# quarterwave0/LithographySimulator

Hardware: AMD Instinct MI355X
Metric: Abbe source-points x image-pixels per second (higher is better)
Workload: dtype f32

## Files before the change

lithographysimulator_amd/csrc/abbe_plan.hpp:

```cpp
#pragma once
#include <climits>
#include <cstddef>
#include <cstdint>
#include <cstdlib>
#include <initializer_list>

#include "../../include/litho_abbe.h"

#ifdef __HIPCC__
#define LITHO_HD __host__ __device__
#else
#define LITHO_HD
#endif

namespace litho {

struct PassGeom {
    int pn, c, N;
    int nt;
    int tcl;
    int kx0, kx1;
    int ky0, ky1;
    int rows;
    int general;
    int rect_off;
    int gcombine;
    int row_pairs;
    int coop_dma;
    unsigned xmask, ymask;
    long long t_point;
};

LITHO_HD constexpr unsigned natural_in_mask(int RL)
{
    return RL == 0 ? 0xF01Fu : RL == 1 ? 0xC007u : RL == 2 ? 0x8003u : 0xFFFFu;
}
LITHO_HD constexpr unsigned out_mask(int RL)
{
    return RL == 1 ? 0xF00Fu : RL == 2 ? 0xC003u : 0xFFFFu;
}

static constexpr int PLAN_WORDS = 14;

static constexpr int COARSE_PLANES = 4;
static constexpr int EDGE_MAX = 128;
static constexpr int GAM_CHUNKS = 1024;
static constexpr size_t GAM_PARTIAL = (size_t)GAM_CHUNKS * 2 * 2 * EDGE_MAX;
static inline size_t gam_float2(int pn) { return GAM_PARTIAL + 2 * 2 * EDGE_MAX + 2 * (size_t)pn; }
static constexpr size_t SIZEOF_FLOAT2 = 8;

struct EdgeGeom {
    int pn, c, h;
    int lo[2], len[2];
};

#ifndef LITHO_G_CAP
#define LITHO_G_CAP 128
#endif
static inline int g_cap(int pn)
{
    const size_t one = (size_t)((pn + 3) / 4) * 4 * pn * sizeof(float);
    size_t n = ((size_t)128 << 20) / one;
    return n < 8 ? 8 : (n > LITHO_G_CAP ? LITHO_G_CAP : (int)n);
}
static constexpr int SLAB_FLUSH_BATCHES = 64;
static constexpr size_t T_BUDGET_MAX = (size_t)1 << 30;
static constexpr size_t T_BUDGET_BIG = (size_t)4 << 30;
static constexpr size_t T_BUDGET_MIN = (size_t)256 << 20;

static inline size_t align_up(size_t v, size_t a) { return (v + a - 1) / a * a; }

static inline size_t general_item_bytes(int pn) { return (size_t)((pn + 3) / 4) * (size_t)pn * 4 * SIZEOF_FLOAT2; }

static inline size_t t_budget(int pn)
{
    const size_t one_general = general_item_bytes(pn);
    size_t b = 64 * one_general;
    if (b < T_BUDGET_MIN) b = T_BUDGET_MIN;
    const size_t cap = pn >= 4096 ? T_BUDGET_BIG : T_BUDGET_MAX;
    if (b > cap) b = cap;
    if (b < one_general + one_general / 2) b = one_general + one_general / 2;
    return b;
}

static inline bool coarse_eligible(int pn, int N)
{
    return N == 2 * pn && (pn == 256 || pn == 512 || pn == 1024 || pn == 2048 || pn == 4096);
}
static inline size_t ic_bytes(int pn, int N) { return coarse_eligible(pn, N) ? (size_t)COARSE_PLANES * pn * pn * sizeof(float) : 0; }
static inline size_t chat_bytes(int pn, int N) { return coarse_eligible(pn, N) ? (size_t)pn * pn * SIZEOF_FLOAT2 : 0; }
static inline size_t gam_bytes(int pn, int N) { return coarse_eligible(pn, N) ? gam_float2(pn) * SIZEOF_FLOAT2 : 0; }

static inline int embedded_size(int pn, int N)
{
    if (pn == N || 2 * pn == N || (pn & 1)) return pn;
    if (2 * pn < N) return N / 2 >= 256 ? N / 2 : pn;
    return N >= 1024 ? N : pn;
}
static inline size_t embed_extra_bytes(int pe)
{
    const size_t e = (size_t)pe * pe;
    return align_up(e * SIZEOF_FLOAT2, 256) + align_up(COARSE_PLANES * e * SIZEOF_FLOAT2, 256) + align_up(COARSE_PLANES * e * sizeof(float), 256);
}

struct Region {
    size_t off, bytes;
    size_t end() const { return off + bytes; }
};
struct WsLayout {
    Region plan;
    Region twtab;
    Region twtab2;
    Region slab;
    Region ic;
    Region chat;
    Region gam;
    Region T;
    size_t total;
};
static inline WsLayout ws_layout(int pn, int N)
{
    const size_t nt = (pn + 3) / 4;
    WsLayout l;
    size_t p = 0;
    l.plan = {p, 256}; p += 256;
    l.twtab = {p, (size_t)N * SIZEOF_FLOAT2}; p += align_up((size_t)N * SIZEOF_FLOAT2, 256);
    l.twtab2 = {p, (size_t)pn * SIZEOF_FLOAT2}; p += align_up((size_t)pn * SIZEOF_FLOAT2, 256);
    l.slab = {p, (size_t)g_cap(pn) * nt * 4 * pn * sizeof(float)}; p += align_up(l.slab.bytes, 256);
    l.ic = {p, ic_bytes(pn, N)}; p += align_up(l.ic.bytes, 256);
    l.chat = {p, chat_bytes(pn, N)}; p += align_up(l.chat.bytes, 256);
    l.gam = {p, gam_bytes(pn, N)}; p += align_up(l.gam.bytes, 256);
    l.T = {p, t_budget(pn)}; p += align_up(l.T.bytes, 256);
    l.total = p;
    return l;
}
static inline size_t workspace_bytes_at(int pn, int N) { return ws_layout(pn, N).total; }
static inline size_t workspace_bytes(int pn, int N)
{
    const size_t own = workspace_bytes_at(pn, N);
    const int pe = embedded_size(pn, N);
    if (pe == pn) return own;
    const size_t emb = workspace_bytes_at(pe, N) + embed_extra_bytes(pe);
    return own > emb ? own : emb;
}

static inline int check_sizes(int pn, int N)
{
    if (pn < 2 || pn > 16384 || (pn & 1)) return LITHO_E_ARG;
    if (N < 16 || N > 16384 || (N & (N - 1))) return LITHO_E_ARG;
    if (N < pn) return LITHO_E_NSMALL;
    return LITHO_OK;
}

static inline int ilog2(int v) { int l = 0; while ((1 << l) < v) ++l; return l; }

static inline int env_int(const char* name, int dflt)
{
    const char* e = getenv(name);
    return (e && *e) ? atoi(e) : dflt;
}

struct Knobs {
    int force_generic, force_general, groups, batch, xchunk, tile, w64, w64_8192, w64x, plane_chunk, xsplit, rect, xrect, coarse, gcombine, rowpairs, poison, embed, split, coopdma;
    static int pick(const litho_abbe_options* o, size_t off, const char* name, int dflt)
    {
        if (o && off + sizeof(int32_t) <= (size_t)o->size) {
            const int32_t v = *(const int32_t*)((const unsigned char*)o + off);
            if (v >= 0) return v;
        }
        return env_int(name, dflt);
    }
    static Knobs read(const litho_abbe_options* o)
    {
#define LITHO_KNOB(field, name, dflt) k.field = pick(o, offsetof(litho_abbe_options, field), name, dflt)
        Knobs k;
        LITHO_KNOB(force_generic, "LITHO_ABBE_FORCE_GENERIC", 0);
        LITHO_KNOB(force_general, "LITHO_ABBE_FORCE_GENERAL", 0);
        LITHO_KNOB(groups, "LITHO_ABBE_GROUPS", 0);
        LITHO_KNOB(batch, "LITHO_ABBE_BATCH", 0);
        LITHO_KNOB(xchunk, "LITHO_ABBE_XCHUNK", 0);
        LITHO_KNOB(tile, "LITHO_ABBE_TILE", 0);
        LITHO_KNOB(w64, "LITHO_ABBE_W64", 1);
        LITHO_KNOB(w64_8192, "LITHO_ABBE_W64_8192", 1);
        LITHO_KNOB(w64x, "LITHO_ABBE_W64X", 0);
        LITHO_KNOB(plane_chunk, "LITHO_ABBE_PLANE_CHUNK", 0);
        LITHO_KNOB(xsplit, "LITHO_ABBE_XSPLIT", 1);
        LITHO_KNOB(rect, "LITHO_ABBE_RECT", 1);
        LITHO_KNOB(xrect, "LITHO_ABBE_XRECT", 1);
        LITHO_KNOB(coarse, "LITHO_ABBE_COARSE", 1);
        LITHO_KNOB(gcombine, "LITHO_ABBE_GCOMBINE", 1);
        LITHO_KNOB(rowpairs, "LITHO_ABBE_ROWPAIRS", 0);
        LITHO_KNOB(poison, "LITHO_ABBE_POISON", 0);
// ... 305 lines not shown
```

lithographysimulator_amd/csrc/engine_kernels.hpp:

```cpp
#pragma once
#include <hip/hip_runtime.h>

#include "engine_common.hpp"
#include "abbe_plan.hpp"
#include "fft_core.hpp"
#include "wave_fft.hpp"

namespace litho {

template <int LOG2N>
struct Launch {
    using F = LineFFT<LOG2N, +1>;
    static constexpr int L = (F::T >= 64) ? 1 : 64 / F::T;
    static constexpr int THREADS = F::T * L;
#ifndef LITHO_NBUF
#define LITHO_NBUF 1
#endif
    static constexpr int NBUF = (LOG2N <= 12) ? LITHO_NBUF : 1;
    static constexpr size_t LDS_EXCH = (size_t)L * NBUF * F::LDS_LINE;
    static constexpr size_t LDS_BYTES = sizeof(float2) * (LDS_EXCH + F::LDS_TW);
#ifndef LITHO_WG_PER_CU
#define LITHO_WG_PER_CU 3
#endif
    static constexpr int WG_PER_CU = LOG2N <= 12 ? LITHO_WG_PER_CU : (LOG2N == 13 ? 2 : 1);
    static constexpr int WAVES = (THREADS / 256 > 0 ? THREADS / 256 : 1) * WG_PER_CU;
};


typedef unsigned int u32x2 __attribute__((ext_vector_type(2)));
static constexpr unsigned BUF_OOB = 0xFFFF0000u;

__device__ __forceinline__ __amdgpu_buffer_rsrc_t make_rsrc(const void* base, size_t bytes) {
    return __builtin_amdgcn_make_buffer_rsrc(const_cast<void*>(base), 0, (int)(unsigned)bytes, 0x00020000);
}
__device__ __forceinline__ float2 buf_load_c64(__amdgpu_buffer_rsrc_t r, unsigned off) {
    const u32x2 v = __builtin_amdgcn_raw_buffer_load_b64(r, off, 0, 0);
    return make_float2(__uint_as_float(v.x), __uint_as_float(v.y));
}
#ifndef LITHO_XSTORE_AUX
#define LITHO_XSTORE_AUX 16
#endif
template <int LOG2N> inline constexpr int t_store_aux = LOG2N >= 11 ? LITHO_XSTORE_AUX : 0;
typedef unsigned int u32x4 __attribute__((ext_vector_type(4)));
template <int AUX = 0>
__device__ __forceinline__ void buf_store_c64x2(__amdgpu_buffer_rsrc_t r, unsigned off, float2 a, float2 b) {
    u32x4 w;
    w.x = __float_as_uint(a.x); w.y = __float_as_uint(a.y);
    w.z = __float_as_uint(b.x); w.w = __float_as_uint(b.y);
    __builtin_amdgcn_raw_buffer_store_b128(w, r, off, 0, AUX);
}
template <int AUX = 0>
__device__ __forceinline__ void buf_store_c64(__amdgpu_buffer_rsrc_t r, unsigned off, float2 v) {
    u32x2 w;
    w.x = __float_as_uint(v.x);
    w.y = __float_as_uint(v.y);
    __builtin_amdgcn_raw_buffer_store_b64(w, r, off, 0, AUX);
}

__device__ __forceinline__ unsigned t_offset(const PassGeom& g, unsigned a, unsigned q) {
    return ((((q >> g.tcl) * g.rows + a) << g.tcl) + (q & ((1u << g.tcl) - 1u)));
}

typedef unsigned int uint2v __attribute__((ext_vector_type(2)));

__device__ __forceinline__ void touch_vgpr(float2& v) { asm volatile("" : "+v"(v.x), "+v"(v.y)); }
__device__ __forceinline__ void diag_keep(float2 v, unsigned o) { asm volatile("" ::"v"(v.x), "v"(v.y), "v"(o)); }

__device__ __forceinline__ const float* pack_weights() { return nullptr; }
__device__ __forceinline__ const float* pack_weights(const float* w) { return w; }

template <int LOG2N, int RL, bool PRUNED, int NP, int RP = 1, typename... Wt>
__global__ __launch_bounds__(Launch<LOG2N>::THREADS, (RP == 2 ? Launch<LOG2N>::WAVES / Launch<LOG2N>::WG_PER_CU * 2 : Launch<LOG2N>::WAVES)) void k_xpass_abbe(
    const float2* __restrict__ P, const float2* __restrict__ M, const int* __restrict__ shifts,
    float2* __restrict__ Tbuf, const float2* __restrict__ twtab, PassGeom g, int nb, int chunk, Wt... wts)
{
    constexpr bool WT = sizeof...(Wt) != 0;
    static_assert(sizeof...(Wt) <= 1 && !(WT && RP == 2), "weighted x-pass: one weight list, one row per workgroup (a weighted call ignores the row-pair knob)");
    [[maybe_unused]] const float* weights = pack_weights(wts...);
    using F = LineFFT<LOG2N, +1>;
    using LC = Launch<LOG2N>;
    constexpr unsigned IN = PRUNED ? natural_in_mask(RL) : 0xFFFFu;
    constexpr unsigned OUT = out_mask(RL);
    extern __shared__ __attribute__((aligned(16))) unsigned char smem_raw[];
    float2* smem = reinterpret_cast<float2*>(smem_raw);
    const int lt = threadIdx.x % F::T, lg = threadIdx.x / F::T;
    float2* lds = smem + (size_t)lg * LC::NBUF * F::LDS_LINE;

    typename F::Twiddles tw;
    F::load_twiddles(tw, twtab, lt, smem + LC::LDS_EXCH, threadIdx.x, LC::THREADS);

    static_assert(RP == 1 || (RP == 2 && NP == 1 && LC::L == 1), "row pairs: one plane, one line per workgroup");
    int a;
    if constexpr (LC::L == 1) {
        const int b = blockIdx.x, xcd = b & 7, i = b >> 3;
        a = ((i >> 2) * 32 + xcd * 4 + (i & 3)) * RP;
    } else {
        a = blockIdx.x * LC::L + lg;
    }
    const bool active = a < g.rows;
    const bool active1 = a + 1 < g.rows;
    const int r = g.ky0 + g.c + a;
    const size_t plane_bytes = (size_t)g.pn * g.pn * sizeof(float2);
    const __amdgpu_buffer_rsrc_t rM = make_rsrc(M, plane_bytes);

    unsigned koff[16];
    float2 pv[NP * RP][16];
    static_for<0, 16>([&](auto e_) {
        constexpr int e = decltype(e_)::value;
        if constexpr ((IN >> e) & 1u) {
            int k;
            const bool ok = centred_index(lt + F::T * e, F::N, g.kx0, g.kx1, k) && active;
            koff[e] = ok ? (unsigned)(g.c + k) : BUF_OOB;
        }
    });
    static_for<0, NP * RP>([&](auto p_) {
        constexpr int p = decltype(p_)::value;
        const __amdgpu_buffer_rsrc_t rP = make_rsrc(P + (size_t)(RP == 1 ? p : 0) * g.pn * g.pn, plane_bytes);
        static_for<0, 16>([&](auto e_) {
            constexpr int e = decltype(e_)::value;
            if constexpr ((IN >> e) & 1u)
                pv[p][e] = buf_load_c64(rP, koff[e] != BUF_OOB ? ((unsigned)(r + (RP == 1 ? 0 : p)) * g.pn + koff[e]) * 8u : BUF_OOB);
        });
    });
    unsigned toff[16];
    static_for<0, 16>([&](auto m_) {
        constexpr int m = decltype(m_)::value;
        if constexpr ((OUT >> m) & 1u) {
            int u;
            const bool ok = centred_index(lt + F::T * m, F::N, -g.c, g.pn - g.c, u) && active;
            const unsigned q = (unsigned)(u + g.c);
            toff[m] = ok ? t_offset(g, a, q) * 8u : BUF_OOB;
        }
    });

    const int s_begin = blockIdx.y * chunk;
    const int s_end = min(nb, s_begin + chunk);
    auto load_window = [&](int s, int rr, float2 (&mv)[16]) {
        const int dy = shifts[2 * s], dx = shifts[2 * s + 1];
        const unsigned mrow = (unsigned)(r + rr + dy) * g.pn + dx;
        static_for<0, 16>([&](auto e_) {
            constexpr int e = decltype(e_)::value;
            if constexpr ((IN >> e) & 1u)
#ifdef LITHO_DIAG_XNOLOAD
                mv[e] = make_float2((float)((mrow + koff[e]) & 1023u), 1.0f);
#else
                mv[e] = buf_load_c64(rM, koff[e] != BUF_OOB ? (mrow + koff[e]) * 8u : BUF_OOB);
#endif
        });
    };

    int flip = 0;
    float2 mnext[16];
    [[maybe_unused]] float wnext = 1.f;
    if (s_begin < s_end) load_window(s_begin, 0, mnext);
    if constexpr (WT) { if (s_begin < s_end) wnext = weights[s_begin]; }
    static_for<0, 16>([&](auto e_) {
        constexpr int e = decltype(e_)::value;
        if constexpr ((IN >> e) & 1u) touch_vgpr(mnext[e]);
    });
    const unsigned row1 = active1 ? (8u << g.tcl) : 0x80000000u;
    float2 held[RP == 2 ? 16 : 1];
    const bool hi8 = (threadIdx.x & 8) != 0;
    unsigned offc = 0, offd = 0;
    if constexpr (RP == 2) {
        const unsigned tileb = (unsigned)g.rows * (8u << g.tcl);
        offc = hi8 ? row1 - tileb : 0u;
        offd = hi8 ? 0u : row1 + tileb;
    }
    for (int s = s_begin; s < s_end; ++s) {
        static_for<0, RP>([&](auto rr_) {
            constexpr int rr = decltype(rr_)::value;
            float2 mv[16];
            static_for<0, 16>([&](auto e_) {
                constexpr int e = decltype(e_)::value;
                if constexpr ((IN >> e) & 1u) mv[e] = mnext[e];
            });
            [[maybe_unused]] float amp = 1.f;
            if constexpr (WT) amp = sqrtf(wnext);
#ifndef LITHO_XPASS_NO_PREFETCH
            if constexpr (rr + 1 < RP) load_window(s, rr + 1, mnext);
            else load_window(s + 1 < s_end ? s + 1 : s, 0, mnext);
#else
            if constexpr (rr + 1 < RP) load_window(s, rr + 1, mnext);
            else if (s + 1 < s_end) load_window(s + 1, 0, mnext);
#endif
            if constexpr (WT) {
                wnext = weights[s + 1 < s_end ? s + 1 : s];
                static_for<0, 16>([&](auto e_) {
                    constexpr int e = decltype(e_)::value;
                    if constexpr ((IN >> e) & 1u) mv[e] = make_float2(amp * mv[e].x, amp * mv[e].y);
                });
            }
            static_for<0, NP>([&](auto p_) {
                constexpr int p = decltype(p_)::value;
                float2 x[16];
                static_for<0, 16>([&](auto e_) {
                    constexpr int e = decltype(e_)::value;
                    if constexpr ((IN >> e) & 1u) x[e] = cmul(pv[RP == 1 ? p : rr][e], mv[e]);
                    else x[e] = make_float2(0.f, 0.f);
                });
                F::template run<LC::NBUF>(x, tw, lds, lt, flip);
                const __amdgpu_buffer_rsrc_t rT =
                    make_rsrc(Tbuf + ((size_t)p * nb + s) * g.t_point, (size_t)g.t_point * sizeof(float2));
                if constexpr (RP == 2 && rr == 0) {
                    static_for<0, 16>([&](auto m_) { held[decltype(m_)::value] = x[decltype(m_)::value]; });
                } else {
                    static_for<0, 16>([&](auto m_) {
                        constexpr int m = decltype(m_)::value;
#ifdef LITHO_DIAG_XNOSTORE
                        if constexpr ((OUT >> m) & 1u) diag_keep(x[m], toff[m]);
#elif defined(LITHO_DIAG_XSTORE_L2)
                        if constexpr ((OUT >> m) & 1u) buf_store_c64(rT, toff[m] == BUF_OOB ? BUF_OOB : (toff[m] & 0xFFFFFu), x[m]);
#else
                        if constexpr ((OUT >> m) & 1u) {
                            if constexpr (RP == 2) {
                                if (active) {
                                    const float bx = __uint_as_float(__builtin_amdgcn_update_dpp(0u, __float_as_uint(x[m].x), 0x128, 0xF, 0xF, false));
                                    const float by = __uint_as_float(__builtin_amdgcn_update_dpp(0u, __float_as_uint(x[m].y), 0x128, 0xF, 0xF, false));
                                    buf_store_c64<t_store_aux<LOG2N>>(rT, toff[m] + offc, hi8 ? make_float2(bx, by) : held[m]);
                                    buf_store_c64<t_store_aux<LOG2N>>(rT, toff[m] + offd, hi8 ? held[m] : make_float2(bx, by));
                                }
                            } else {
                                buf_store_c64<t_store_aux<LOG2N>>(rT, toff[m], x[m]);
                            }
                        }
#endif
                    });
                }
            });
        });
    }
}

template <int LOG2N, typename... Wt>
__global__ __launch_bounds__(Launch<LOG2N - 1>::THREADS, Launch<LOG2N - 1>::WAVES) void k_xpass_split(
    const float2* __restrict__ P, const float2* __restrict__ M, const int* __restrict__ shifts,
    float2* __restrict__ Tbuf, const float2* __restrict__ twtab, PassGeom g, int nb, int chunk, Wt... wts)
{
    constexpr bool WT = sizeof...(Wt) != 0;
    static_assert(sizeof...(Wt) <= 1, "one weight list");
    [[maybe_unused]] const float* weights = pack_weights(wts...);
    using F = LineFFT<LOG2N - 1, +1>;
    using LC = Launch<LOG2N - 1>;
    static_assert(LC::L == 1, "split x-pass: one row per workgroup");
    constexpr unsigned IN = natural_in_mask(0), OUT = out_mask(1);
    extern __shared__ __attribute__((aligned(16))) unsigned char smem_raw[];
    float2* smem = reinterpret_cast<float2*>(smem_raw);
    const int lt = threadIdx.x;
    float2* lds = smem;

    typename F::Twiddles tw;
    F::load_twiddles(tw, twtab, lt, smem + LC::LDS_EXCH, threadIdx.x, LC::THREADS, 2);

    const int b = blockIdx.x, xcd = b & 7, i = b >> 3;
    const int a = (i >> 2) * 32 + xcd * 4 + (i & 3);
    const bool active = a < g.rows;
    const int r = g.ky0 + g.c + a;
    const size_t plane_bytes = (size_t)g.pn * g.pn * sizeof(float2);
    const __amdgpu_buffer_rsrc_t rM = make_rsrc(M, plane_bytes);
    const __amdgpu_buffer_rsrc_t rP = make_rsrc(P, plane_bytes);

    unsigned koff[16];
    float2 pv0[16], pv1[16];
    static_for<0, 16>([&](auto e_) {
        constexpr int e = decltype(e_)::value;
        if constexpr ((IN >> e) & 1u) {
            int k;
            const bool ok = centred_index(lt + F::T * e, F::N, g.kx0, g.kx1, k) && active;
            koff[e] = ok ? (unsigned)(g.c + k) : BUF_OOB;
            pv0[e] = buf_load_c64(rP, ok ? ((unsigned)r * g.pn + koff[e]) * 8u : BUF_OOB);
            pv1[e] = cmul(pv0[e], twtab[(k + 2 * F::N) & (2 * F::N - 1)]);
        }
    });
    unsigned toff[16];
    static_for<0, 16>([&](auto m_) {
        constexpr int m = decltype(m_)::value;
        if constexpr ((OUT >> m) & 1u) {
            int v;
            const bool ok = centred_index(lt + F::T * m, F::N, -(g.c >> 1), g.c >> 1, v) && active;
            toff[m] = ok ? t_offset(g, a, (unsigned)(2 * v + g.c)) * 8u : BUF_OOB;
        }
    });

    const int s_begin = blockIdx.y * chunk;
    const int s_end = min(nb, s_begin + chunk);
    int flip = 0;
    for (int s = s_begin; s < s_end; ++s) {
        const int dy = shifts[2 * s], dx = shifts[2 * s + 1];
        const unsigned mrow = (unsigned)(r + dy) * g.pn + dx;
        float2 mv[16];
        static_for<0, 16>([&](auto e_) {
            constexpr int e = decltype(e_)::value;
            if constexpr ((IN >> e) & 1u) mv[e] = buf_load_c64(rM, koff[e] != BUF_OOB ? (mrow + koff[e]) * 8u : BUF_OOB);
        });
        if constexpr (WT) {
            const float amp = sqrtf(weights[s]);
            static_for<0, 16>([&](auto e_) {
                constexpr int e = decltype(e_)::value;
                if constexpr ((IN >> e) & 1u) mv[e] = make_float2(amp * mv[e].x, amp * mv[e].y);
            });
        }
        float2 x[16], even[16];
        static_for<0, 16>([&](auto e_) {
            constexpr int e = decltype(e_)::value;
            if constexpr ((IN >> e) & 1u) x[e] = cmul(pv0[e], mv[e]);
            else x[e] = make_float2(0.f, 0.f);
        });
        F::template run<LC::NBUF>(x, tw, lds, lt, flip);
        static_for<0, 16>([&](auto m_) {
            constexpr int m = decltype(m_)::value;
            if constexpr ((OUT >> m) & 1u) even[m] = x[m];
        });
        static_for<0, 16>([&](auto e_) {
            constexpr int e = decltype(e_)::value;
            if constexpr ((IN >> e) & 1u) x[e] = cmul(pv1[e], mv[e]);
            else x[e] = make_float2(0.f, 0.f);
        });
        F::template run<LC::NBUF>(x, tw, lds, lt, flip);
        const __amdgpu_buffer_rsrc_t rT =
            make_rsrc(Tbuf + (size_t)s * g.t_point, (size_t)g.t_point * sizeof(float2));
        static_for<0, 16>([&](auto m_) {
            constexpr int m = decltype(m_)::value;
            if constexpr ((OUT >> m) & 1u) buf_store_c64x2<t_store_aux<LOG2N>>(rT, toff[m], even[m], x[m]);
        });
    }
}

template <int LOG2N, int SIGN, typename Loader>
__global__ __launch_bounds__(Launch<LOG2N>::THREADS, Launch<LOG2N>::WAVES) void k_xpass(
    Loader ld, float2* __restrict__ Tbuf, const float2* __restrict__ twtab, PassGeom g)
{
    using F = LineFFT<LOG2N, SIGN>;
    using LC = Launch<LOG2N>;
    extern __shared__ __attribute__((aligned(16))) unsigned char smem_raw[];
    float2* smem = reinterpret_cast<float2*>(smem_raw);
    const int lt = threadIdx.x % F::T, lg = threadIdx.x / F::T;
    float2* lds = smem + (size_t)lg * LC::NBUF * F::LDS_LINE;

    typename F::Twiddles tw;
    F::load_twiddles(tw, twtab, lt, smem + LC::LDS_EXCH, threadIdx.x, LC::THREADS);

    const int s = blockIdx.y;
    const int a = blockIdx.x * LC::L + lg;
    const bool active = a < g.rows;
    ld.begin_line(s, active ? a : 0, g);

    float2 x[16];
#pragma unroll
    for (int e = 0; e < 16; ++e) {
        int k;
        const bool ok = centred_index(lt + F::T * e, F::N, g.kx0, g.kx1, k) && active;
        x[e] = ok ? ld.load(k, g) : make_float2(0.f, 0.f);
    }
    int flip = 0;
    F::template run<LC::NBUF>(x, tw, lds, lt, flip);

    float2* tpt = Tbuf + (size_t)s * g.t_point;
#pragma unroll
    for (int m = 0; m < 16; ++m) {
        int u;
        if (centred_index(lt + F::T * m, F::N, -g.c, g.pn - g.c, u) && active) {
            tpt[t_offset(g, a, (unsigned)(u + g.c))] = x[m];
        }
    }
}

struct AbbeLoader {
    const float2* P;
    const float2* M;
    const int* shifts;
    const float2* prow;
    const float2* mrow;
    int dx, pad_;
    __device__ __forceinline__ void begin_line(int s, int a, const PassGeom& g) {
        const int dy = shifts[2 * s];
        dx = shifts[2 * s + 1];
        if (!g.general) {
            const int r = g.ky0 + g.c + a;
            prow = P + (size_t)r * g.pn;
            mrow = M + (size_t)(r + dy) * g.pn + dx;
        } else {
            int r = (a - dy) % g.pn;
            if (r < 0) r += g.pn;
            prow = P + (size_t)r * g.pn;
// ... 168 lines not shown
    int cur_group = -1, a = 0, r = 0;
    bool active = false;
    for (int it = i0; it < i1; ++it) {
        const int grp = it / nb, s = it - grp * nb;
        if (grp != cur_group) {
            cur_group = grp;
            a = grp * 4 + wv;
            active = a < g.rows;
            r = g.ky0 + g.c + (active ? a : 0);
            const __amdgpu_buffer_rsrc_t rP = make_rsrc(P + (size_t)r * g.pn + g.c + g.kx0, active ? win_bytes : 0u);
            static_for<0, 64>([&](auto j_) {
                constexpr int j = decltype(j_)::value;
                if constexpr (j <= 8 || j >= 56) pv[j] = buf_load_c64(rP, slot_off(j));
            });
        }
        if (!active) continue;
        const int dy = shifts[2 * s], dx = shifts[2 * s + 1];
        const __amdgpu_buffer_rsrc_t rM = make_rsrc(M + (size_t)(r + dy) * g.pn + dx + g.c + g.kx0, win_bytes);
        float2 x[64];
        static_for<0, 64>([&](auto j_) {
            constexpr int j = decltype(j_)::value;
            if constexpr (j <= 8 || j >= 56) x[j] = cmul(pv[j], buf_load_c64(rM, slot_off(j)));
            else x[j] = make_float2(0.f, 0.f);
        });
        Wave4096::run(x, tw, lds, lane);
        const __amdgpu_buffer_rsrc_t rT =
            make_rsrc(Tbuf + (size_t)s * g.t_point, (size_t)g.t_point * sizeof(float2));
        const unsigned vbase = (((unsigned)(lane >> 2) * g.rows + a) * 4u + (lane & 3u)) * 8u;
        const unsigned kstride = 16u * g.rows * 32u;
        static_for<0, 32>([&](auto i_) {
            constexpr int i = decltype(i_)::value;
            constexpr int k2 = i < 16 ? i : 32 + i;
            constexpr int kk = i < 16 ? i + 16 : i - 16;
#ifdef LITHO_DIAG_XNOSTORE
            diag_keep(x[Wave4096::brev(k2)], vbase + kk * kstride);
#else
            buf_store_c64(rT, vbase + kk * kstride, x[Wave4096::brev(k2)]);
#endif
        });
    }
}

template <int LOG2N, int SIGN>
__global__ __launch_bounds__(Launch<LOG2N>::THREADS, Launch<LOG2N>::WAVES) void k_ypass_field(
    const float2* __restrict__ Tbuf, float2* __restrict__ field, const float2* __restrict__ twtab, PassGeom g)
{
    using F = LineFFT<LOG2N, SIGN>;
    using LC = Launch<LOG2N>;
    extern __shared__ __attribute__((aligned(16))) unsigned char smem_raw[];
    float2* smem = reinterpret_cast<float2*>(smem_raw);
    const int lt = threadIdx.x % F::T, lg = threadIdx.x / F::T;
    float2* lds = smem + (size_t)lg * LC::NBUF * F::LDS_LINE;
    typename F::Twiddles tw;
    F::load_twiddles(tw, twtab, lt, smem + LC::LDS_EXCH, threadIdx.x, LC::THREADS);
    const int tile = blockIdx.x * LC::L + lg;
    const bool active = tile < g.nt;
    int flip = 0;
    for (int cidx = 0; cidx < 4; ++cidx) {
        float2 x[16];
#pragma unroll
        for (int e = 0; e < 16; ++e) {
            int k;
            const bool ok = centred_index(lt + F::T * e, F::N, g.ky0, g.ky1, k) && active;
            x[e] = ok ? Tbuf[t_offset(g, (unsigned)(k - g.ky0), (unsigned)tile * 4u + cidx)] : make_float2(0.f, 0.f);
        }
        F::template run<LC::NBUF>(x, tw, lds, lt, flip);
        const int qx = tile * 4 + cidx;
        if (!active || qx >= g.pn) continue;
#pragma unroll
        for (int m = 0; m < 16; ++m) {
            int u;
            if (centred_index(lt + F::T * m, F::N, -g.c, g.pn - g.c, u)) field[(size_t)(u + g.c) * g.pn + qx] = x[m];
        }
    }
}

template <int LOG2N>
__global__ __launch_bounds__(Launch<LOG2N>::THREADS, Launch<LOG2N>::WAVES) void k_ypass_addreal(
    const float2* __restrict__ Tbuf, float* __restrict__ img, float scale, const float2* __restrict__ twtab, PassGeom g)
{
    using F = LineFFT<LOG2N, +1>;
    using LC = Launch<LOG2N>;
    extern __shared__ __attribute__((aligned(16))) unsigned char smem_raw[];
    float2* smem = reinterpret_cast<float2*>(smem_raw);
    const int lt = threadIdx.x % F::T, lg = threadIdx.x / F::T;
    float2* lds = smem + (size_t)lg * LC::NBUF * F::LDS_LINE;
    typename F::Twiddles tw;
    F::load_twiddles(tw, twtab, lt, smem + LC::LDS_EXCH, threadIdx.x, LC::THREADS);
    const int tile = blockIdx.x * LC::L + lg;
    const bool active = tile < g.nt;
    int flip = 0;
    for (int cidx = 0; cidx < 4; ++cidx) {
        float2 x[16];
#pragma unroll
        for (int e = 0; e < 16; ++e) {
            int k;
            const bool ok = centred_index(lt + F::T * e, F::N, g.ky0, g.ky1, k) && active;
            x[e] = ok ? Tbuf[t_offset(g, (unsigned)(k - g.ky0), (unsigned)tile * 4u + cidx)] : make_float2(0.f, 0.f);
        }
        F::template run<LC::NBUF>(x, tw, lds, lt, flip);
        const int qx = tile * 4 + cidx;
        if (!active || qx >= g.pn) continue;
#pragma unroll
        for (int m = 0; m < 16; ++m) {
            int u;
            if (centred_index(lt + F::T * m, F::N, -g.c, g.pn - g.c, u)) img[(size_t)(u + g.c) * g.pn + qx] += scale * x[m].x;
        }
    }
}

struct SizeOps {
    hipError_t (*xpass_abbe)(int variant, int np, const float2* P, const float2* M, const int* shifts, const float* wts, float2* T,
                             const float2* tw, const PassGeom& g, int nb, int chunk, hipStream_t st);
    hipError_t (*xpass_general)(const AbbeLoader& ld, const float* wts, float2* T, const float2* tw, const PassGeom& g, int nb,
                                hipStream_t st);
    hipError_t (*xpass_split)(const float2* P, const float2* M, const int* shifts, const float* wts, float2* T, const float2* tw,
                              const PassGeom& g, int nb, int chunk, hipStream_t st);
    hipError_t (*xpass_rect)(const float2* P, const float2* M, const int* shifts, const float* wts, float2* T, const float2* tw,
                             const PassGeom& g, int nb, int chunk, hipStream_t st);
    hipError_t (*xpass_real_fwd)(const RealImageLoader& ld, float2* T, const float2* tw, const PassGeom& g,
                                 hipStream_t st);
    hipError_t (*ypass_acc)(int variant, const float2* T, float* slab, const float2* tw, const PassGeom& g, int nb,
                            int planes, int G, int gstride, hipStream_t st);
    hipError_t (*ypass_field)(int sign, const float2* T, float2* field, const float2* tw, const PassGeom& g,
                              hipStream_t st);
    hipError_t (*xpass_field_inv)(const FieldLoader& ld, float2* T, const float2* tw, const PassGeom& g, hipStream_t st);
    hipError_t (*ypass_addreal)(const float2* T, float* img, float scale, const float2* tw, const PassGeom& g,
                                hipStream_t st);
    hipError_t (*xpass_w64)(const float2* P, const float2* M, const int* shifts, float2* T, const float2* tw,
                            const PassGeom& g, int nb, hipStream_t st);
    hipError_t (*ypass_w64)(const float2* T, float* slab, const float2* tw, const PassGeom& g, int nb, int planes,
                            int G, int gstride, hipStream_t st);
    hipError_t (*xpass_cplx_fwd)(const ComplexImageLoader& ld, float2* T, const float2* tw, const PassGeom& g,
                                 hipStream_t st);
};
const SizeOps* size_ops(int log2n);

struct LdsOnce {
    unsigned done = 0;
};
template <typename K>
static hipError_t set_lds(LdsOnce& once, K kern, size_t bytes)
{
    int dev = 0;
    hipError_t e = hipGetDevice(&dev);
    if (e != hipSuccess) return e;
    const unsigned bit = 1u << (dev & 31);
    if (__atomic_load_n(&once.done, __ATOMIC_ACQUIRE) & bit) return hipSuccess;
    e = hipFuncSetAttribute((const void*)kern, hipFuncAttributeMaxDynamicSharedMemorySize, (int)bytes);
    if (e == hipSuccess) __atomic_fetch_or(&once.done, bit, __ATOMIC_RELEASE);
    return e;
}

template <int LOG2N>
hipError_t launch_ypass_wave(const float2* T, float* slab, const float2* tw, const PassGeom& g, int nb, int planes,
                             int G, int gstride, hipStream_t st);

template <int LOG2N>
hipError_t launch_xpass_rect(const float2* P, const float2* M, const int* shifts, const float* wts, float2* T, const float2* tw,
                             const PassGeom& g, int nb, int chunk, hipStream_t st);

template <int LOG2N>
struct SizeImpl {
    using LC = Launch<LOG2N>;

    template <int RL, bool PRUNED, int NP, int RP = 1>
    static hipError_t xa(const float2* P, const float2* M, const int* shifts, const float* wts, float2* T, const float2* tw,
                         const PassGeom& g, int nb, int chunk, hipStream_t st)
    {
        if (wts) {
            if constexpr (RP == 1) {
                static LdsOnce once_wt;
                auto kern = k_xpass_abbe<LOG2N, RL, PRUNED, NP, 1, const float*>;
                hipError_t e = set_lds(once_wt, kern, LC::LDS_BYTES);
                if (e != hipSuccess) return e;
                dim3 grid(LC::L == 1 ? (g.rows + 31) / 32 * 32 : (g.rows + LC::L - 1) / LC::L, (nb + chunk - 1) / chunk);
                hipLaunchKernelGGL(kern, grid, dim3(LC::THREADS), LC::LDS_BYTES, st, P, M, shifts, T, tw, g, nb, chunk, wts);
                note_kernel(0, PRUNED ? "k_xpass_abbe<%d, %d, true, %d, 1, float const*>" : "k_xpass_abbe<%d, %d, false, %d, 1, float const*>", LOG2N, RL, NP);
                return hipGetLastError();
            } else {
                return hipErrorInvalidValue;
            }
        }
        static LdsOnce once;
        auto kern = k_xpass_abbe<LOG2N, RL, PRUNED, NP, RP>;
        hipError_t e = set_lds(once, kern, LC::LDS_BYTES);
        if (e != hipSuccess) return e;
        const int wrows = (g.rows + RP - 1) / RP;
        dim3 grid(LC::L == 1 ? (wrows + 31) / 32 * 32 : (wrows + LC::L - 1) / LC::L, (nb + chunk - 1) / chunk);
        hipLaunchKernelGGL(kern, grid, dim3(LC::THREADS), LC::LDS_BYTES, st, P, M, shifts, T, tw, g, nb, chunk);
        note_kernel(0, PRUNED ? "k_xpass_abbe<%d, %d, true, %d, %d>" : "k_xpass_abbe<%d, %d, false, %d, %d>", LOG2N, RL, NP, RP);
        return hipGetLastError();
    }
    template <int RL>
    static hipError_t xa_np(int np, const float2* P, const float2* M, const int* shifts, const float* wts, float2* T, const float2* tw,
                            const PassGeom& g, int nb, int chunk, hipStream_t st)
    {
        if constexpr (LOG2N == 12 && RL == 0) {
            if (np == 1 && g.row_pairs) return xa<RL, true, 1, 2>(P, M, shifts, wts, T, tw, g, nb, chunk, st);
        }
        if (np == 1) return xa<RL, true, 1>(P, M, shifts, wts, T, tw, g, nb, chunk, st);
        if constexpr (RL >= 1) {
            if (np == 2) return xa<RL, true, 2>(P, M, shifts, wts, T, tw, g, nb, chunk, st);
            if (np == 4) return xa<RL, true, 4>(P, M, shifts, wts, T, tw, g, nb, chunk, st);
        }
        return hipErrorInvalidValue;
    }
    static hipError_t xpass_abbe(int variant, int np, const float2* P, const float2* M, const int* shifts, const float* wts, float2* T,
                                 const float2* tw, const PassGeom& g, int nb, int chunk, hipStream_t st)
    {
        switch (variant) {
            case 0: return xa_np<0>(np, P, M, shifts, wts, T, tw, g, nb, chunk, st);
            case 1: return xa_np<1>(np, P, M, shifts, wts, T, tw, g, nb, chunk, st);
            case 2: return xa_np<2>(np, P, M, shifts, wts, T, tw, g, nb, chunk, st);
            default:
                if (np != 1) return hipErrorInvalidValue;
                return xa<-1, false, 1>(P, M, shifts, wts, T, tw, g, nb, chunk, st);
        }
    }
    static hipError_t xpass_general(const AbbeLoader& ld, const float* wts, float2* T, const float2* tw, const PassGeom& g, int nb,
                                    hipStream_t st)
    {
        if (wts) {
            static LdsOnce once_wt;
            auto kern = k_xpass<LOG2N, +1, AbbeLoaderW>;
            hipError_t e = set_lds(once_wt, kern, LC::LDS_BYTES);
            if (e != hipSuccess) return e;
            AbbeLoaderW lw{ld, wts, 1.f, 0.f};
            hipLaunchKernelGGL(kern, dim3((g.rows + LC::L - 1) / LC::L, nb), dim3(LC::THREADS), LC::LDS_BYTES, st, lw, T,
                               tw, g);
            note_kernel(0, "k_xpass<%d, 1, litho::AbbeLoaderW>", LOG2N);
            return hipGetLastError();
        }
        static LdsOnce once;
        auto kern = k_xpass<LOG2N, +1, AbbeLoader>;
        hipError_t e = set_lds(once, kern, LC::LDS_BYTES);
        if (e != hipSuccess) return e;
        hipLaunchKernelGGL(kern, dim3((g.rows + LC::L - 1) / LC::L, nb), dim3(LC::THREADS), LC::LDS_BYTES, st, ld, T,
                           tw, g);
        note_kernel(0, "k_xpass<%d, 1, litho::AbbeLoader>", LOG2N);
        return hipGetLastError();
    }
    static hipError_t xpass_split(const float2* P, const float2* M, const int* shifts, const float* wts, float2* T, const float2* tw,
                                  const PassGeom& g, int nb, int chunk, hipStream_t st)
    {
        if constexpr (LOG2N == 13) {
            using LH = Launch<LOG2N - 1>;
            if (wts) {
                static LdsOnce once_wt;
                auto kern = k_xpass_split<LOG2N, const float*>;
                hipError_t e = set_lds(once_wt, kern, LH::LDS_BYTES);
                if (e != hipSuccess) return e;
                dim3 grid((g.rows + 31) / 32 * 32, (nb + chunk - 1) / chunk);
                hipLaunchKernelGGL(kern, grid, dim3(LH::THREADS), LH::LDS_BYTES, st, P, M, shifts, T, tw, g, nb, chunk, wts);
                note_kernel(0, "k_xpass_split<%d, float const*>", LOG2N);
                return hipGetLastError();
            }
            static LdsOnce once;
            auto kern = k_xpass_split<LOG2N>;
            hipError_t e = set_lds(once, kern, LH::LDS_BYTES);
            if (e != hipSuccess) return e;
            dim3 grid((g.rows + 31) / 32 * 32, (nb + chunk - 1) / chunk);
            hipLaunchKernelGGL(kern, grid, dim3(LH::THREADS), LH::LDS_BYTES, st, P, M, shifts, T, tw, g, nb, chunk);
            note_kernel(0, "k_xpass_split<%d>", LOG2N);
            return hipGetLastError();
        } else {
            return hipErrorNotSupported;
        }
    }
    static hipError_t xpass_rect(const float2* P, const float2* M, const int* shifts, const float* wts, float2* T, const float2* tw,
                                 const PassGeom& g, int nb, int chunk, hipStream_t st)
    {
        if constexpr (LOG2N >= 9 && LOG2N <= 13) return launch_xpass_rect<LOG2N>(P, M, shifts, wts, T, tw, g, nb, chunk, st);
        else return hipErrorNotSupported;
    }
    static hipError_t xpass_real_fwd(const RealImageLoader& ld, float2* T, const float2* tw, const PassGeom& g,
                                     hipStream_t st)
    {
        static LdsOnce once;
        auto kern = k_xpass<LOG2N, -1, RealImageLoader>;
        hipError_t e = set_lds(once, kern, LC::LDS_BYTES);
        if (e != hipSuccess) return e;
        hipLaunchKernelGGL(kern, dim3((g.rows + LC::L - 1) / LC::L, 1), dim3(LC::THREADS), LC::LDS_BYTES, st, ld, T, tw,
                           g);
        return hipGetLastError();
    }
    static hipError_t xpass_cplx_fwd(const ComplexImageLoader& ld, float2* T, const float2* tw, const PassGeom& g,
                                     hipStream_t st)
    {
        static LdsOnce once;
        auto kern = k_xpass<LOG2N, -1, ComplexImageLoader>;
        hipError_t e = set_lds(once, kern, LC::LDS_BYTES);
        if (e != hipSuccess) return e;
        hipLaunchKernelGGL(kern, dim3((g.rows + LC::L - 1) / LC::L, 1), dim3(LC::THREADS), LC::LDS_BYTES, st, ld, T, tw,
                           g);
        return hipGetLastError();
    }
    template <int RL, bool PRUNED>
    static hipError_t ya(const float2* T, float* slab, const float2* tw, const PassGeom& g, int nb, int planes, int G,
                         int gstride, hipStream_t st)
    {
        static LdsOnce once;
        auto kern = k_ypass_acc<LOG2N, RL, PRUNED>;
        hipError_t e = set_lds(once, kern, LC::LDS_BYTES);
        if (e != hipSuccess) return e;
        hipLaunchKernelGGL(kern, dim3((g.nt + LC::L - 1) / LC::L, planes * G), dim3(LC::THREADS), LC::LDS_BYTES, st, T,
                           slab, tw, g, nb, G, gstride);
        note_kernel(1, PRUNED ? "k_ypass_acc<%d, %d, true>" : "k_ypass_acc<%d, %d, false>", LOG2N, RL);
        return hipGetLastError();
    }
    static hipError_t ypass_acc(int variant, const float2* T, float* slab, const float2* tw, const PassGeom& g, int nb,
                                int planes, int G, int gstride, hipStream_t st)
    {
        switch (variant) {
            case 0: return ya<0, true>(T, slab, tw, g, nb, planes, G, gstride, st);
            case 1: return ya<1, true>(T, slab, tw, g, nb, planes, G, gstride, st);
            case 2: return ya<2, true>(T, slab, tw, g, nb, planes, G, gstride, st);
            default: return ya<-1, false>(T, slab, tw, g, nb, planes, G, gstride, st);
        }
    }
    static hipError_t xpass_field_inv(const FieldLoader& ld, float2* T, const float2* tw, const PassGeom& g, hipStream_t st)
    {
        static LdsOnce once;
        auto kern = k_xpass<LOG2N, +1, FieldLoader>;
        hipError_t e = set_lds(once, kern, LC::LDS_BYTES);
        if (e != hipSuccess) return e;
        hipLaunchKernelGGL(kern, dim3((g.rows + LC::L - 1) / LC::L, 1), dim3(LC::THREADS), LC::LDS_BYTES, st, ld, T, tw, g);
        return hipGetLastError();
    }
    static hipError_t ypass_addreal(const float2* T, float* img, float scale, const float2* tw, const PassGeom& g,
                                    hipStream_t st)
    {
        static LdsOnce once;
        auto kern = k_ypass_addreal<LOG2N>;
        hipError_t e = set_lds(once, kern, LC::LDS_BYTES);
        if (e != hipSuccess) return e;
        hipLaunchKernelGGL(kern, dim3((g.nt + LC::L - 1) / LC::L), dim3(LC::THREADS), LC::LDS_BYTES, st, T, img, scale, tw, g);
        return hipGetLastError();
    }
    static hipError_t xpass_w64(const float2* P, const float2* M, const int* shifts, float2* T, const float2* tw,
                                const PassGeom& g, int nb, hipStream_t st)
    {
// ... 58 lines not shown
```

Baseline: 495.2 billion.

## Balance x-pass work across XCDs with persistent occupancy-sized grid

For single-line workgroups without row pairs, the x-pass now launches a 1-D grid sized from the resident workgroup capacity. Each workgroup walks a contiguous range of (row, source-point) items inside its XCD's row partition and loops over row segments. This replaces the fixed rows x chunks 2-D grid and is meant to remove tail imbalance and idle workgroups for out-of-range rows. In exchange it recomputes row setup (P loads, offsets) whenever a workgroup crosses into a new row, and it adds an occupancy query on first launch.

```diff
diff --git a/lithographysimulator_amd/csrc/abbe_plan.hpp b/lithographysimulator_amd/csrc/abbe_plan.hpp
--- a/lithographysimulator_amd/csrc/abbe_plan.hpp
+++ b/lithographysimulator_amd/csrc/abbe_plan.hpp
@@ -38,6 +38,38 @@
 LITHO_HD constexpr unsigned out_mask(int RL)
 {
     return RL == 1 ? 0xF00Fu : RL == 2 ? 0xC003u : 0xFFFFu;
+}
+
+static constexpr int XPART_XCDS = 8;
+LITHO_HD constexpr int xpart_rows(int rows, int x)
+{
+    const int rem = rows % 32 - 4 * x;
+    return rows / 32 * 4 + (rem < 0 ? 0 : rem > 4 ? 4 : rem);
+}
+LITHO_HD constexpr int xpart_row(int x, int i) { return (i >> 2) * 32 + x * 4 + (i & 3); }
+struct XRange {
+    int begin, end;
+};
+LITHO_HD constexpr XRange xpart_range(int rows, int nb, int W, int w)
+{
+    const int n = xpart_rows(rows, w % XPART_XCDS) * nb, wx = W / XPART_XCDS, i = w / XPART_XCDS;
+    const int base = n / wx, extra = n % wx;
+    const int begin = i * base + (i < extra ? i : extra);
+    return XRange{begin, begin + base + (i < extra ? 1 : 0)};
+}
+static inline int xpart_grid(int rows, int nb, int chunk, int slots)
+{
+    const long long items = (long long)rows * nb;
+    if (chunk < 1) chunk = 1;
+    if (slots < XPART_XCDS) slots = XPART_XCDS;
+    slots -= slots % XPART_XCDS;
+    const long long target = (items + chunk - 1) / chunk;
+    if (target >= slots) {
+        const long long rounds = (2 * target + slots) / (2 * slots);
+        return (int)(slots * rounds);
+    }
+    const long long w = (target + XPART_XCDS - 1) / XPART_XCDS * XPART_XCDS;
+    return (int)(w < XPART_XCDS ? XPART_XCDS : w);
 }
 
 static constexpr int PLAN_WORDS = 14;
diff --git a/lithographysimulator_amd/csrc/engine_kernels.hpp b/lithographysimulator_amd/csrc/engine_kernels.hpp
--- a/lithographysimulator_amd/csrc/engine_kernels.hpp
+++ b/lithographysimulator_amd/csrc/engine_kernels.hpp
@@ -63,6 +63,12 @@
 
 typedef unsigned int uint2v __attribute__((ext_vector_type(2)));
 
+#if defined(LITHO_DIAG_XGRID_LEGACY) || defined(LITHO_DIAG_XGRID_DROPROW)
+inline constexpr bool XPASS_LEGACY_GRID = true;
+#else
+inline constexpr bool XPASS_LEGACY_GRID = false;
+#endif
+
 __device__ __forceinline__ void touch_vgpr(float2& v) { asm volatile("" : "+v"(v.x), "+v"(v.y)); }
 __device__ __forceinline__ void diag_keep(float2 v, unsigned o) { asm volatile("" ::"v"(v.x), "v"(v.y), "v"(o)); }
 
@@ -86,22 +92,45 @@
     const int lt = threadIdx.x % F::T, lg = threadIdx.x / F::T;
     float2* lds = smem + (size_t)lg * LC::NBUF * F::LDS_LINE;
 
+    static_assert(RP == 1 || (RP == 2 && NP == 1 && LC::L == 1), "row pairs: one plane, one line per workgroup");
+    constexpr bool BAL = LC::L == 1 && RP == 1 && !XPASS_LEGACY_GRID;
+    [[maybe_unused]] int it = 0, it_end = 0, xcd = 0;
+    int a = 0;
+    if constexpr (BAL) {
+        const XRange rg = xpart_range(g.rows, nb, (int)gridDim.x, (int)blockIdx.x);
+        if (rg.begin >= rg.end) return;
+        it = rg.begin; it_end = rg.end; xcd = blockIdx.x & 7;
+    } else if constexpr (LC::L == 1) {
+        const int b = blockIdx.x, x = b & 7, i = b >> 3;
+        a = ((i >> 2) * 32 + x * 4 + (i & 3)) * RP;
+        if (a >= g.rows) return;
+    } else {
+        a = blockIdx.x * LC::L + lg;
+    }
+
     typename F::Twiddles tw;
     F::load_twiddles(tw, twtab, lt, smem + LC::LDS_EXCH, threadIdx.x, LC::THREADS);
 
-    static_assert(RP == 1 || (RP == 2 && NP == 1 && LC::L == 1), "row pairs: one plane, one line per workgroup");
-    int a;
-    if constexpr (LC::L == 1) {
-        const int b = blockIdx.x, xcd = b & 7, i = b >> 3;
-        a = ((i >> 2) * 32 + xcd * 4 + (i & 3)) * RP;
+    const size_t plane_bytes = (size_t)g.pn * g.pn * sizeof(float2);
+    const __amdgpu_buffer_rsrc_t rM = make_rsrc(M, plane_bytes);
+    int flip = 0;
+    do {
+    int s_begin, s_end;
+    if constexpr (BAL) {
+        const int lr = it / nb;
+        a = xpart_row(xcd, lr);
+        s_begin = it - lr * nb;
+        s_end = min(nb, s_begin + (it_end - it));
+        it += s_end - s_begin;
     } else {
-        a = blockIdx.x * LC::L + lg;
-    }
-    const bool active = a < g.rows;
+        s_begin = blockIdx.y * chunk;
+        s_end = min(nb, s_begin + chunk);
+    }
+    const bool active = BAL || a < g.rows;
     const bool active1 = a + 1 < g.rows;
     const int r = g.ky0 + g.c + a;
-    const size_t plane_bytes = (size_t)g.pn * g.pn * sizeof(float2);
-    const __amdgpu_buffer_rsrc_t rM = make_rsrc(M, plane_bytes);
+    int lts = lt;
+    if constexpr (BAL) asm volatile("" : "+v"(lts));
 
     unsigned koff[16];
     float2 pv[NP * RP][16];
@@ -109,7 +138,7 @@
         constexpr int e = decltype(e_)::value;
         if constexpr ((IN >> e) & 1u) {
             int k;
-            const bool ok = centred_index(lt + F::T * e, F::N, g.kx0, g.kx1, k) && active;
+            const bool ok = centred_index(lts + F::T * e, F::N, g.kx0, g.kx1, k) && active;
             koff[e] = ok ? (unsigned)(g.c + k) : BUF_OOB;
         }
     });
@@ -127,14 +156,12 @@
         constexpr int m = decltype(m_)::value;
         if constexpr ((OUT >> m) & 1u) {
             int u;
-            const bool ok = centred_index(lt + F::T * m, F::N, -g.c, g.pn - g.c, u) && active;
+            const bool ok = centred_index(lts + F::T * m, F::N, -g.c, g.pn - g.c, u) && active;
             const unsigned q = (unsigned)(u + g.c);
             toff[m] = ok ? t_offset(g, a, q) * 8u : BUF_OOB;
         }
     });
 
-    const int s_begin = blockIdx.y * chunk;
-    const int s_end = min(nb, s_begin + chunk);
     auto load_window = [&](int s, int rr, float2 (&mv)[16]) {
         const int dy = shifts[2 * s], dx = shifts[2 * s + 1];
         const unsigned mrow = (unsigned)(r + rr + dy) * g.pn + dx;
@@ -149,7 +176,6 @@
         });
     };
 
-    int flip = 0;
     float2 mnext[16];
     [[maybe_unused]] float wnext = 1.f;
     if (s_begin < s_end) load_window(s_begin, 0, mnext);
@@ -230,6 +256,7 @@
             });
         });
     }
+    } while (BAL && it < it_end);
 }
 
 template <int LOG2N, typename... Wt>
@@ -704,6 +731,28 @@
     return e;
 }
 
+struct SlotsOnce {
+    int slots[32] = {};
+};
+template <typename K>
+static hipError_t resident_slots(SlotsOnce& once, K kern, int threads, size_t lds_bytes, int& out)
+{
+    int dev = 0;
+    hipError_t e = hipGetDevice(&dev);
+    if (e != hipSuccess) return e;
+    int& slot = once.slots[dev & 31];
+    out = __atomic_load_n(&slot, __ATOMIC_ACQUIRE);
+    if (out > 0) return hipSuccess;
+    int per_cu = 0, cus = 0;
+    e = hipOccupancyMaxActiveBlocksPerMultiprocessor(&per_cu, (const void*)kern, threads, lds_bytes);
+    if (e != hipSuccess) return e;
+    e = hipDeviceGetAttribute(&cus, hipDeviceAttributeMultiprocessorCount, dev);
+    if (e != hipSuccess) return e;
+    out = (per_cu > 0 ? per_cu : 1) * (cus > 0 ? cus : 1);
+    __atomic_store_n(&slot, out, __ATOMIC_RELEASE);
+    return hipSuccess;
+}
+
 template <int LOG2N>
 hipError_t launch_ypass_wave(const float2* T, float* slab, const float2* tw, const PassGeom& g, int nb, int planes,
                              int G, int gstride, hipStream_t st);
@@ -716,6 +765,24 @@
 struct SizeImpl {
     using LC = Launch<LOG2N>;
 
+    template <int RP, typename K>
+    static hipError_t xa_grid(SlotsOnce& slots, K kern, const PassGeom& g, int nb, int chunk, dim3& grid)
+    {
+        if constexpr (LC::L == 1 && RP == 1 && !XPASS_LEGACY_GRID) {
+            int n = 0;
+            const hipError_t e = resident_slots(slots, kern, LC::THREADS, LC::LDS_BYTES, n);
+            if (e != hipSuccess) return e;
+            grid = dim3(xpart_grid(g.rows, nb, chunk, n));
+        } else {
+#ifdef LITHO_DIAG_XGRID_DROPROW
+            const int wrows = LC::L == 1 && g.rows > 1 ? g.rows - 1 : g.rows;
+#else
+            const int wrows = (g.rows + RP - 1) / RP;
+#endif
+            grid = dim3(LC::L == 1 ? (wrows + 31) / 32 * 32 : (wrows + LC::L - 1) / LC::L, (nb + chunk - 1) / chunk);
+        }
+        return hipSuccess;
+    }
     template <int RL, bool PRUNED, int NP, int RP = 1>
     static hipError_t xa(const float2* P, const float2* M, const int* shifts, const float* wts, float2* T, const float2* tw,
                          const PassGeom& g, int nb, int chunk, hipStream_t st)
@@ -723,10 +790,13 @@
         if (wts) {
             if constexpr (RP == 1) {
                 static LdsOnce once_wt;
+                static SlotsOnce slots_wt;
                 auto kern = k_xpass_abbe<LOG2N, RL, PRUNED, NP, 1, const float*>;
                 hipError_t e = set_lds(once_wt, kern, LC::LDS_BYTES);
                 if (e != hipSuccess) return e;
-                dim3 grid(LC::L == 1 ? (g.rows + 31) / 32 * 32 : (g.rows + LC::L - 1) / LC::L, (nb + chunk - 1) / chunk);
+                dim3 grid;
+                e = xa_grid<1>(slots_wt, kern, g, nb, chunk, grid);
+                if (e != hipSuccess) return e;
                 hipLaunchKernelGGL(kern, grid, dim3(LC::THREADS), LC::LDS_BYTES, st, P, M, shifts, T, tw, g, nb, chunk, wts);
                 note_kernel(0, PRUNED ? "k_xpass_abbe<%d, %d, true, %d, 1, float const*>" : "k_xpass_abbe<%d, %d, false, %d, 1, float const*>", LOG2N, RL, NP);
                 return hipGetLastError();
@@ -735,11 +805,13 @@
             }
         }
         static LdsOnce once;
+        static SlotsOnce slots;
         auto kern = k_xpass_abbe<LOG2N, RL, PRUNED, NP, RP>;
         hipError_t e = set_lds(once, kern, LC::LDS_BYTES);
         if (e != hipSuccess) return e;
-        const int wrows = (g.rows + RP - 1) / RP;
-        dim3 grid(LC::L == 1 ? (wrows + 31) / 32 * 32 : (wrows + LC::L - 1) / LC::L, (nb + chunk - 1) / chunk);
+        dim3 grid;
+        e = xa_grid<RP>(slots, kern, g, nb, chunk, grid);
+        if (e != hipSuccess) return e;
         hipLaunchKernelGGL(kern, grid, dim3(LC::THREADS), LC::LDS_BYTES, st, P, M, shifts, T, tw, g, nb, chunk);
         note_kernel(0, PRUNED ? "k_xpass_abbe<%d, %d, true, %d, %d>" : "k_xpass_abbe<%d, %d, false, %d, %d>", LOG2N, RL, NP, RP);
         return hipGetLastError();
```

Result: no change. 496.0 billion, median of 2 (+0.2%).
